# ai4co/rl4co

Hardware: NVIDIA H100
Metric: node-selections/sec TSP-100 AM rollout (higher is better)
Workload: dtype f32

## Files before the change

rl4co_b200/csrc/rollout_impl.cuh:

```cuda
#pragma once
#include "co_common.cuh"

namespace co {

#define CO_MODE_GREEDY 0
#define CO_MODE_SAMPLE 1
#define CO_MODE_EVALUATE 2

template <int SPL>
struct Cfg {
  static constexpr int NS = 32 * SPL;
  static constexpr int NW = SPL;
  static constexpr int MINB = SPL == 4 ? 1 : (SPL == 2 ? 2 : 3);
};

constexpr int TILE_LD = 20;

template <int SPL>
struct Smem {
  float ptab[(32 * SPL + 1) * E];
  float qfix[E];
  float wcap[E];
  float hfirst[E];
  float tile[8][32 * TILE_LD];
  alignas(16) float oh[8][D];
  alignas(16) float part[8][32 * SPL];
  alignas(16) float zbuf[2][32 * SPL];
  alignas(16) uint2 red[4];
  alignas(16) float lps[32];
  float dem[32 * SPL];
  float lim[32 * SPL];
  float2 loc[32 * SPL];
  unsigned char order[32 * SPL];
  unsigned char rank_of[32 * SPL];
  alignas(16) float wdyn[3 * E];
  alignas(16) float pwk[32 * SPL * 8 + 8];
};

__device__ __forceinline__ float ex2(float x) {
  float y;
  asm("ex2.approx.ftz.f32 %0, %1;" : "=f"(y) : "f"(x));
  return y;
}
__device__ __forceinline__ float lg2(float x) {
  float y;
  asm("lg2.approx.ftz.f32 %0, %1;" : "=f"(y) : "f"(x));
  return y;
}
__device__ __forceinline__ unsigned fkey(float f) {
  unsigned u = __float_as_uint(f);
  return u ^ ((u >> 31) ? 0xffffffffu : 0x80000000u);
}
__device__ __forceinline__ float funkey(unsigned k) {
  return __uint_as_float(k ^ ((k >> 31) ? 0x80000000u : 0xffffffffu));
}

__device__ __forceinline__ float warp_sum_fixed(float x) {
  constexpr float S = 16777216.f;
  const unsigned hi = __float2uint_rz(x * S);
  const float rem = fmaf(x, S, -(float)hi);
  const unsigned lo = __float2uint_rz(rem * S);
  const unsigned Hs = __reduce_add_sync(FULL, hi), Ls = __reduce_add_sync(FULL, lo);
  return fmaf((float)Ls, 1.0f / (S * S), (float)Hs * (1.0f / S));
}

static __device__ __noinline__ void first_node_gemv(const float* __restrict__ w_first, const float* hfirst, float* qfix, int tid) {
  const int e = tid >> 1, half = tid & 1;
  const float4* wr = reinterpret_cast<const float4*>(w_first + (size_t)e * E + 64 * half);
  const float4* hv = reinterpret_cast<const float4*>(hfirst + 64 * half);
  float s0 = 0.f, s1 = 0.f;
#pragma unroll
  for (int c = 0; c < 16; c += 2) {
    const float4 w0 = __ldg(wr + c), x0 = hv[c], w1 = __ldg(wr + c + 1), x1 = hv[c + 1];
    s0 = fmaf(w0.x, x0.x, s0); s0 = fmaf(w0.y, x0.y, s0); s0 = fmaf(w0.z, x0.z, s0); s0 = fmaf(w0.w, x0.w, s0);
    s1 = fmaf(w1.x, x1.x, s1); s1 = fmaf(w1.y, x1.y, s1); s1 = fmaf(w1.z, x1.z, s1); s1 = fmaf(w1.w, x1.w, s1);
  }
  float sacc = s0 + s1;
  sacc += __shfl_xor_sync(FULL, sacc, 1);
  if (half == 0) qfix[e] += sacc;
}

__device__ __forceinline__ float dist2_fma(float2 a, float2 b) {
  const float dx = a.x - b.x, dy = a.y - b.y;
  return sqrtf(fmaf(dy, dy, dx * dx));
}

template <int ENV>
__device__ __forceinline__ bool feasible(int n, bool visbit, float d, float used, float thr, int cur, bool anyfeas) {
  if (ENV == CO_ENV_TSP) return !visbit;
  if (ENV == CO_ENV_OP) return (n == 0) || (!visbit && !anyfeas && !(d > thr));
  if (ENV == CO_ENV_PCTSP) return (n == 0) ? !((used < 1.0f) && anyfeas) : (!visbit && d == 0.0f);
  if (n == 0) return !(cur == 0 && anyfeas);
  if (ENV == CO_ENV_SDVRP) return !visbit && !(d == 0.0f) && !(used >= thr);
  return !visbit && !((d + used) > thr);
}

template <int SPL, int ENV, int MODE, int CWB>
__global__ void __launch_bounds__(256, Cfg<SPL>::MINB) rollout_kernel(const co_rollout_args A) {
  using C = Cfg<SPL>;
  constexpr int NS = C::NS, NW = C::NW;
  constexpr int CW = CWB * E;
  constexpr int CUR_BLK = CWB - 1;
  constexpr bool first_table = (ENV == CO_ENV_TSP) && (CWB == 5);
  constexpr bool VRP = (ENV != CO_ENV_TSP);
  constexpr bool SD = (ENV == CO_ENV_SDVRP);
  constexpr bool OP = (ENV == CO_ENV_OP);
  constexpr bool PC = (ENV == CO_ENV_PCTSP);
  constexpr float LOG2E = 1.4426950408889634f, LN2 = 0.6931471805599453f;
  extern __shared__ __align__(16) unsigned char smem_raw[];
  Smem<SPL>& sm = *reinterpret_cast<Smem<SPL>*>(smem_raw);

  const int tid = threadIdx.x, lane = tid & 31, h = tid >> 5;
  const int N = A.N, B_inst = A.B_inst, S = A.num_starts, T_max = A.T_max;
  const int B_traj = B_inst * S;
  const bool forced_start = (S > 1) && (A.flags & CO_ROLLOUT_FORCED_START);
  const bool philox = (A.noise == nullptr);
  const bool sel_warp = h < NW;
  const bool lp_warp = h == NW;
  const int nL = sel_warp ? tid : NS - 1;
  const int nG = SPL * lane;
  const float clip = A.tanh_clipping, inv_temp = 1.0f / A.temperature;
  const float Zb = clip * inv_temp;
  float* tile = sm.tile[h];

  float2 Kr[SPL][8], Vr[SPL][8], Lr[SPL][8];

  for (int b = blockIdx.x; b < B_inst; b += gridDim.x) {
    __syncthreads();
    const float* crow = A.cache + (size_t)b * N * CW;
#pragma unroll
    for (int k = 0; k < SPL; ++k) {
      const int n = nG + k;
      if (n < N) {
        const float4* ks = reinterpret_cast<const float4*>(crow + (size_t)n * CW + 0 * E + h * D);
        const float4* vs = reinterpret_cast<const float4*>(crow + (size_t)n * CW + 1 * E + h * D);
        const float4* ls = reinterpret_cast<const float4*>(crow + (size_t)n * CW + 2 * E + h * D);
#pragma unroll
        for (int c = 0; c < 4; ++c) {
          const float4 kv = __ldg(ks + c), vv = __ldg(vs + c), lv = __ldg(ls + c);
          Kr[k][2 * c] = make_float2(kv.x, kv.y); Kr[k][2 * c + 1] = make_float2(kv.z, kv.w);
          Vr[k][2 * c] = make_float2(vv.x, vv.y); Vr[k][2 * c + 1] = make_float2(vv.z, vv.w);
          Lr[k][2 * c] = make_float2(lv.x, lv.y); Lr[k][2 * c + 1] = make_float2(lv.z, lv.w);
        }
      } else {
#pragma unroll
        for (int j = 0; j < 8; ++j) {
          Kr[k][j] = make_float2(0.f, 0.f); Vr[k][j] = make_float2(0.f, 0.f); Lr[k][j] = make_float2(0.f, 0.f);
        }
      }
    }
    for (int idx = tid; idx < N * (E / 4); idx += 256) {
      const int n = idx >> 5, c = idx & 31;
      const uint32_t dst = (uint32_t)__cvta_generic_to_shared(reinterpret_cast<float4*>(sm.ptab + n * E) + c);
      asm volatile("cp.async.cg.shared.global [%0], [%1], 16;" ::"r"(dst),
                   "l"(reinterpret_cast<const float4*>(crow + (size_t)n * CW + CUR_BLK * E) + c) : "memory");
    }
    asm volatile("cp.async.commit_group;" ::: "memory");
    if (tid < E) {
      sm.ptab[NS * E + tid] = 0.f;
      sm.wcap[tid] = VRP ? A.w_capacity[tid] : 0.f;
    }
    if (tid < NS) {
      sm.loc[tid] = (tid < N) ? reinterpret_cast<const float2*>(A.locs)[(size_t)b * N + tid] : make_float2(0.f, 0.f);
      sm.dem[tid] = (VRP && tid >= 1 && tid < N) ? A.demand[(size_t)b * (N - 1) + tid - 1] : 0.f;
      if (OP || PC) sm.lim[tid] = (tid < N) ? A.node_limit[(size_t)b * N + tid] : 0.f;
    }
    if (SD) {
      for (int i = tid; i < 3 * E; i += 256) sm.wdyn[i] = A.dyn_w[i];
    }
    const float cap = (VRP && A.vehicle_capacity) ? A.vehicle_capacity[b] : 1.0f;
    const float thr = SD ? cap : cap + 1e-5f;
    asm volatile("cp.async.wait_group 0;" ::: "memory");
    __syncthreads();
    if (SD) {
      for (int i = tid; i < (NS + 1) * 8; i += 256) {
        const int n = i >> 3, hh = i & 7;
        float acc = 0.f;
        if (n < N) {
#pragma unroll
          for (int c = 0; c < D; ++c) acc = fmaf(sm.ptab[n * E + hh * D + c], sm.wdyn[hh * D + c], acc);
        }
        sm.pwk[i] = acc;
      }
      __syncthreads();
    }
    if (ENV == CO_ENV_CVRP) {
      if (tid >= 1 && tid < N) {
        const float d = sm.dem[tid];
        int rank = 0;
        for (int m = 1; m < N; ++m) {
          const float dm = sm.dem[m];
          rank += (dm < d || (dm == d && m < tid)) ? 1 : 0;
        }
        sm.order[rank] = (unsigned char)tid;
        sm.rank_of[tid] = (unsigned char)rank;
      }
      __syncthreads();
    }
    float dmk0[SPL];
    float2 lck[SPL];
#pragma unroll
    for (int k = 0; k < SPL; ++k) {
      dmk0[k] = OP ? sm.lim[nG + k] : sm.dem[nG + k];
      lck[k] = OP ? sm.loc[nG + k] : make_float2(0.f, 0.f);
    }
    const float dL0 = OP ? sm.lim[nL] : sm.dem[nL];
    const float2 lcL = OP ? sm.loc[nL] : make_float2(0.f, 0.f);
    auto head_dot = [&](const float* vec, float (&out)[SPL]) {
      const float4* vp = reinterpret_cast<const float4*>(vec + h * D);
      float2 a2[SPL];
#pragma unroll
      for (int k = 0; k < SPL; ++k) a2[k] = make_float2(0.f, 0.f);
#pragma unroll
      for (int c = 0; c < 4; ++c) {
        const float4 x = vp[c];
#pragma unroll
        for (int k = 0; k < SPL; ++k) {
          a2[k] = ffma2(make_float2(x.x, x.y), Kr[k][2 * c], a2[k]);
          a2[k] = ffma2(make_float2(x.z, x.w), Kr[k][2 * c + 1], a2[k]);
        }
      }
#pragma unroll
      for (int k = 0; k < SPL; ++k) out[k] = a2[k].x + a2[k].y;
    };
    auto add_first = [&](int a_first) {
      if (first_table) {
        if (tid < E) sm.qfix[tid] += __ldg(crow + (size_t)a_first * CW + 3 * E + tid);
      } else {
        if (tid < E) sm.hfirst[tid] = __ldg(A.node_emb + ((size_t)b * N + a_first) * E + tid);
        __syncthreads();
        first_node_gemv(A.w_first, sm.hfirst, sm.qfix, tid);
      }
    };
    float WK[SPL], FK[SPL];
#pragma unroll
    for (int k = 0; k < SPL; ++k) { WK[k] = 0.f; FK[k] = 0.f; }
    if (VRP) head_dot(sm.wcap, WK);
    float WKW = 0.f, wv_d = 0.f;
    if (SD) {
#pragma unroll
      for (int c = 0; c < D; ++c) WKW = fmaf(sm.wcap[h * D + c], sm.wdyn[h * D + c], WKW);
      wv_d = sm.wdyn[E + h * D + (lane & 15)];
    }
    if (!(A.flags & CO_ROLLOUT_NO_PREFETCH) && b + (int)gridDim.x < B_inst) {
      const char* nxt = reinterpret_cast<const char*>(A.cache + (size_t)(b + gridDim.x) * N * CW);
      for (int i = tid; i < N * 16; i += 256) {
        const int n = i >> 4, blk = (i >> 2) & 3, line = i & 3;
        const size_t off = ((size_t)n * CW + (blk < 3 ? blk : CUR_BLK) * E) * 4 + ((size_t)line << 7);
        asm volatile("prefetch.global.L2 [%0];" ::"l"(nxt + off));
      }
    }

    for (int s = 0; s < S; ++s) {
      const int traj = s * B_inst + b;
      int64_t* act_row = A.actions_out + (size_t)traj * T_max;
      float* lp_row = A.logp_out + (size_t)traj * T_max;
      uint32_t mybits = (!sel_warp || nL >= N) ? 0x100u : 0u;
#pragma unroll
      for (int k = 0; k < SPL; ++k) mybits |= (nG + k >= N) ? (1u << k) : 0u;
      int cur = (ENV == CO_ENV_TSP) ? NS : 0;
      int prev = 0, first = 0, t = 0, dstep = 0, nvis = 0;
      uint32_t rmask[SPL];
#pragma unroll
      for (int k = 0; k < SPL; ++k) {
        const int lo = 32 * k, nc = N - 1;
        rmask[k] = (nc >= lo + 32) ? 0u : (nc <= lo ? 0xffffffffu : (0xffffffffu << (nc - lo)));
      }
      float used = 0.f, dist = 0.f;
      bool anyfeas = false, done = false, depot_seen = false;
      float dmk[SPL], dL = dL0;
#pragma unroll
      for (int k = 0; k < SPL; ++k) dmk[k] = dmk0[k];
      int nrem = 0;
      int pend_a = -1;
      float pend_d = 0.f, FKW = 0.f;
      float ll = 0.f;
      float pen = 0.f;
      if (SD && s > 0 && tid < NS) sm.dem[tid] = (tid >= 1 && tid < N) ? A.demand[(size_t)b * (N - 1) + tid - 1] : 0.f;
      __syncthreads();
      if (tid < E) {
        float g = A.graph_ctx ? A.graph_ctx[(size_t)b * E + tid] : 0.f;
        if (ENV == CO_ENV_TSP && !forced_start) g += A.q_placeholder[tid];
        sm.qfix[tid] = g;
      }

      auto env_step = [&](int a) {
        if (!SD) {
          const unsigned dd = (unsigned)(a - nG);
          mybits |= (dd < (unsigned)SPL) ? (1u << dd) : 0u;
          mybits |= (a == nL) ? 0x100u : 0u;
        }
        if (!OP && h == 0) {
          const float2 pa = sm.loc[a], pp = sm.loc[prev];
          const float dx = pa.x - pp.x, dy = pa.y - pp.y;
          if (VRP || t != 0) dist += sqrtf(dx * dx + dy * dy);
        }
        if (ENV == CO_ENV_TSP) {
          if (t == 0) first = a;
        } else if (OP) {
          used = used + dist2_fma(sm.loc[a], sm.loc[prev]);
          if (h == 0) dist += sm.dem[a];
          depot_seen = depot_seen || (a == 0);
        } else if (PC) {
          used = used + sm.dem[a];
          if (h == 0) pen += sm.lim[a];
          nvis += (a != 0) ? 1 : 0;
          depot_seen = depot_seen || (a == 0);
        } else if (SD) {
          const float d_a = sm.dem[a];
          const float delivered = fminf(d_a, cap - used);
          used = (used + delivered) * (a != 0 ? 1.0f : 0.0f);
          const float d_new = d_a + (-delivered);
#pragma unroll
          for (int k = 0; k < SPL; ++k) dmk[k] = (a == nG + k) ? d_new : dmk[k];
          dL = (a == nL) ? d_new : dL;
          nrem += ((d_new > 0.f) ? 1 : 0) - ((d_a > 0.f) ? 1 : 0);
          pend_a = a; pend_d = d_new;
          anyfeas = (nrem > 0) && !(used >= cap);
        } else {
          used = (used + sm.dem[a == 0 ? 1 : a]) * (a != 0 ? 1.0f : 0.0f);
          nvis += (a != 0 || !depot_seen) ? 1 : 0;
          depot_seen = depot_seen || (a == 0);
          if (a != 0) {
            const int r = sm.rank_of[a];
#pragma unroll
            for (int k = 0; k < SPL; ++k) rmask[k] |= ((r >> 5) == k) ? (1u << (r & 31)) : 0u;
          }
          int pmin = NS;
#pragma unroll
          for (int k = SPL - 1; k >= 0; --k) {
            const uint32_t z = ~rmask[k];
            if (z) pmin = 32 * k + __ffs(z) - 1;
          }
          anyfeas = (pmin < N - 1) && !((sm.dem[sm.order[pmin < N - 1 ? pmin : 0]] + used) > thr);
        }
        prev = a; cur = a; ++t;
        done = (ENV == CO_ENV_TSP) ? (t >= N) : ((OP || PC) ? (a == 0 && t > 1) : (SD ? (nrem == 0) : (nvis >= N)));
      };
      auto logp_of = [&](int buf, int a_sel, int t_out) {
        const float* zb = sm.zbuf[buf];
        float sacc = 0.f;
#pragma unroll
        for (int k = 0; k < SPL; ++k) sacc += ex2((zb[nG + k] - Zb) * LOG2E);
        sm.lps[lane] = sacc;
        __syncwarp();
        const float4* lq = reinterpret_cast<const float4*>(sm.lps);
        const float4 q0 = lq[0], q1 = lq[1], q2 = lq[2], q3 = lq[3], q4 = lq[4], q5 = lq[5], q6 = lq[6], q7 = lq[7];
        const float t0 = ((q0.x + q0.y) + (q0.z + q0.w)) + ((q1.x + q1.y) + (q1.z + q1.w));
        const float t1 = ((q2.x + q2.y) + (q2.z + q2.w)) + ((q3.x + q3.y) + (q3.z + q3.w));
        const float t2 = ((q4.x + q4.y) + (q4.z + q4.w)) + ((q5.x + q5.y) + (q5.z + q5.w));
        const float t3 = ((q6.x + q6.y) + (q6.z + q6.w)) + ((q7.x + q7.y) + (q7.z + q7.w));
        sacc = (t0 + t1) + (t2 + t3);
        __syncwarp();
        const float lp = (zb[a_sel] - Zb) - lg2(sacc) * LN2;
        if (lane == 0) {
          lp_row[t_out] = lp;
          ll += lp;
        }
      };

      if (SD) {
        for (int n = 1; n < N; ++n) nrem += (sm.dem[n] > 0.f) ? 1 : 0;
        anyfeas = (nrem > 0) && !(used >= cap);
        done = (nrem == 0);
      }
      if (forced_start) {
        const int a0 = (s % A.num_loc) + (VRP ? 1 : 0);
        if (tid == 0) { act_row[0] = a0; lp_row[0] = 0.f; }
        env_step(a0);
        if (ENV == CO_ENV_TSP) {
          __syncthreads();
          add_first(a0);
        }
      } else if (ENV == CO_ENV_CVRP) {
        anyfeas = !((sm.dem[sm.order[0]] + used) > thr);
      }
      __syncthreads();
      head_dot(sm.qfix, FK);
      if (SD) {
#pragma unroll
        for (int c = 0; c < D; ++c) FKW = fmaf(sm.qfix[h * D + c], sm.wdyn[h * D + c], FKW);
      }

      while (!done && t < T_max) {
        int forced = 0;
        float gum = 0.f;
        if (MODE == CO_MODE_EVALUATE) forced = (int)A.forced_actions[(size_t)traj * T_max + t];
        if (MODE == CO_MODE_SAMPLE && tid < N) {
          const float q = philox ? philox_exp1(A.seed, A.offset, traj, dstep, tid)
                                 : A.noise[((size_t)dstep * B_traj + traj) * N + tid];
          gum = -logf(q);
        }

        {
          const float4* pr = reinterpret_cast<const float4*>(sm.ptab + cur * E + h * D);
          const float rem = PC ? fmaxf(cap - used, 0.0f) : cap - used;
          float2 sc2[SPL];
#pragma unroll
          for (int k = 0; k < SPL; ++k) sc2[k] = make_float2(0.f, 0.f);
#pragma unroll
          for (int c = 0; c < 4; ++c) {
            const float4 p = pr[c];
#pragma unroll
            for (int k = 0; k < SPL; ++k) {
              sc2[k] = ffma2(make_float2(p.x, p.y), Kr[k][2 * c], sc2[k]);
              sc2[k] = ffma2(make_float2(p.z, p.w), Kr[k][2 * c + 1], sc2[k]);
            }
          }
          float sc[SPL], m = -INFINITY;
          bool fz[SPL];
          const float qwk = SD ? fmaf(rem, WKW, sm.pwk[cur * 8 + h] + FKW) : 0.f;
          const float2 pcur = OP ? sm.loc[cur] : make_float2(0.f, 0.f);
#pragma unroll
          for (int k = 0; k < SPL; ++k) {
            fz[k] = OP ? feasible<ENV>(nG + k, (mybits >> k) & 1u, used + dist2_fma(lck[k], pcur), used, dmk[k], cur, depot_seen)
                    : PC ? feasible<ENV>(nG + k, (mybits >> k) & 1u, depot_seen ? 1.0f : 0.0f, used, thr, cur, nvis < N - 1)
                         : feasible<ENV>(nG + k, (mybits >> k) & 1u, dmk[k], used, thr, cur, anyfeas);
            float dot = (sc2[k].x + sc2[k].y) + FK[k];
            if (VRP) dot = fmaf(rem, WK[k], dot);
            if (SD) dot = fmaf(dmk[k], qwk, dot);
            sc[k] = fz[k] ? dot * (0.25f * LOG2E) : -INFINITY;
            m = fmaxf(m, sc[k]);
          }
          m = funkey(__reduce_max_sync(FULL, fkey(m)));
          float2 acc[8];
          float esum = 0.f, sed = 0.f;
#pragma unroll
          for (int j = 0; j < 8; ++j) acc[j] = make_float2(0.f, 0.f);
#pragma unroll
          for (int k = 0; k < SPL; ++k) {
            const float e = fz[k] ? ex2(sc[k] - m) : 0.f;
            esum += e;
            if (SD) sed = fmaf(e, dmk[k], sed);
            const float2 e2 = make_float2(e, e);
#pragma unroll
            for (int j = 0; j < 8; ++j) acc[j] = ffma2(e2, Vr[k][j], acc[j]);
          }
          float4* trow = reinterpret_cast<float4*>(tile + lane * TILE_LD);
#pragma unroll
          for (int c = 0; c < 4; ++c) trow[c] = make_float4(acc[2 * c].x, acc[2 * c].y, acc[2 * c + 1].x, acc[2 * c + 1].y);
          if (SD) sed = warp_sum(sed);
          __syncwarp();
          const int d = lane & 15, half = lane >> 4;
          float s0 = 0.f, s1 = 0.f, s2 = 0.f, s3 = 0.f;
#pragma unroll
          for (int r = 0; r < 16; r += 4) {
            s0 += tile[(16 * half + ((r + 0 + 4 * half) & 15)) * TILE_LD + d];
            s1 += tile[(16 * half + ((r + 1 + 4 * half) & 15)) * TILE_LD + d];
            s2 += tile[(16 * half + ((r + 2 + 4 * half) & 15)) * TILE_LD + d];
            s3 += tile[(16 * half + ((r + 3 + 4 * half) & 15)) * TILE_LD + d];
          }
          float r = (s0 + s1) + (s2 + s3);
          r += __shfl_xor_sync(FULL, r, 16);
          if (SD) r = fmaf(sed, wv_d, r);
          if (lane < 16) sm.oh[h][lane] = r;
          __syncwarp();
          const float4* op = reinterpret_cast<const float4*>(sm.oh[h]);
          float2 pl2[SPL];
          float olh = 0.f;
#pragma unroll
          for (int k = 0; k < SPL; ++k) pl2[k] = make_float2(0.f, 0.f);
#pragma unroll
          for (int c = 0; c < 4; ++c) {
            const float4 x = op[c];
#pragma unroll
            for (int k = 0; k < SPL; ++k) {
              pl2[k] = ffma2(make_float2(x.x, x.y), Lr[k][2 * c], pl2[k]);
              pl2[k] = ffma2(make_float2(x.z, x.w), Lr[k][2 * c + 1], pl2[k]);
            }
            if (SD) {
              const float4 w = reinterpret_cast<const float4*>(sm.wdyn + 2 * E + h * D)[c];
              olh = fmaf(x.x, w.x, olh); olh = fmaf(x.y, w.y, olh); olh = fmaf(x.z, w.z, olh); olh = fmaf(x.w, w.w, olh);
            }
          }
          esum = warp_sum_fixed(esum);
          const float rinv = __fdividef(1.0f, esum);
          float pl[SPL];
#pragma unroll
          for (int k = 0; k < SPL; ++k) {
            float v = pl2[k].x + pl2[k].y;
            if (SD) v = fmaf(dmk[k], olh, v);
            pl[k] = v * rinv;
          }
          float* pdst = sm.part[h] + nG;
          if (SPL == 4) *reinterpret_cast<float4*>(pdst) = make_float4(pl[0], pl[SPL > 1 ? 1 : 0], pl[SPL > 2 ? 2 : 0], pl[SPL > 3 ? 3 : 0]);
          else if (SPL == 2) *reinterpret_cast<float2*>(pdst) = make_float2(pl[0], pl[SPL > 1 ? 1 : 0]);
          else *pdst = pl[0];
        }
        __syncthreads();

        if (SD && tid == 0 && pend_a >= 0) sm.dem[pend_a] = pend_d;
        if (sel_warp) {
          const bool fzL = OP ? feasible<ENV>(nL, (mybits >> 8) & 1u, used + dist2_fma(lcL, sm.loc[cur]), used, dL, cur, depot_seen)
                           : PC ? feasible<ENV>(nL, (mybits >> 8) & 1u, depot_seen ? 1.0f : 0.0f, used, thr, cur, nvis < N - 1)
                                : feasible<ENV>(nL, (mybits >> 8) & 1u, dL, used, thr, cur, anyfeas);
          const float p = ((sm.part[0][nL] + sm.part[1][nL]) + (sm.part[2][nL] + sm.part[3][nL])) +
                          ((sm.part[4][nL] + sm.part[5][nL]) + (sm.part[6][nL] + sm.part[7][nL]));
          const float lg = tanhf(p * 0.08838834764831845f) * clip;
          const float z = fzL ? lg * inv_temp : -INFINITY;
          sm.zbuf[dstep & 1][nL] = z;
          if (MODE != CO_MODE_EVALUATE) {
            const float keyf = (MODE == CO_MODE_SAMPLE) ? (fzL ? z + gum : -INFINITY) : z;
            const unsigned key = fkey(keyf);
            const unsigned wkey = __reduce_max_sync(FULL, key);
            const unsigned vote = __ballot_sync(FULL, key == wkey);
            if (lane == 0) sm.red[h] = make_uint2(wkey, (unsigned)(32 * h + __ffs(vote) - 1));
          }
        } else if (lp_warp && dstep > 0) {
          logp_of((dstep - 1) & 1, prev, t - 1);
        }
        __syncthreads();
        int a;
        if (MODE == CO_MODE_EVALUATE) {
          a = (forced < 0 || forced >= N) ? 0 : forced;
        } else if (NW == 1) {
          a = (int)sm.red[0].y;
        } else if (NW == 2) {
          const uint4 r0 = reinterpret_cast<const uint4*>(sm.red)[0];
          a = (int)((r0.z > r0.x) ? r0.w : r0.y);
        } else {
          const uint4 r0 = reinterpret_cast<const uint4*>(sm.red)[0], r1 = reinterpret_cast<const uint4*>(sm.red)[1];
          const bool b01 = r0.z > r0.x, b23 = r1.z > r1.x;
          const unsigned ka = b01 ? r0.z : r0.x, ia = b01 ? r0.w : r0.y;
          const unsigned kb = b23 ? r1.z : r1.x, ib = b23 ? r1.w : r1.y;
          a = (int)((kb > ka) ? ib : ia);
        }
        if (tid == 0) act_row[t] = a;

        const bool was_first = (ENV == CO_ENV_TSP) && (t == 0);
        env_step(a);
        ++dstep;
        if (was_first) {
          if (tid < E) sm.qfix[tid] = A.graph_ctx ? A.graph_ctx[(size_t)b * E + tid] : 0.f;
          __syncthreads();
          add_first(a);
          __syncthreads();
          head_dot(sm.qfix, FK);
        }
      }

      __syncthreads();
      if (lp_warp) {
        if (dstep > 0) logp_of((dstep - 1) & 1, prev, t - 1);
        if (lane == 0) A.loglik_out[traj] = ll;
      }
      if (tid == 0) {
        const float2 pa = sm.loc[(ENV == CO_ENV_TSP) ? first : 0], pp = sm.loc[prev];
        const float dx = pa.x - pp.x, dy = pa.y - pp.y;
        float rw = OP ? dist : -(dist + sqrtf(dx * dx + dy * dy));
        if (PC) {
          float total = 0.f;
          for (int n = 1; n < N; ++n) total += sm.lim[n];
          rw = pen - (-rw + total);
        }
        A.reward_out[traj] = rw;
        if (A.steps_out) A.steps_out[traj] = t;
        if (A.used_capacity_out) A.used_capacity_out[traj] = used;
        if (A.max_steps_out) atomicMax(A.max_steps_out, t);
      }
      for (int c = t + tid; c < T_max; c += 256) { act_row[c] = 0; lp_row[c] = 0.f; }
    }
  }
}

template <int SPL, int ENV, int MODE, int CWB>
static int launch(const co_rollout_args& A, cudaStream_t st) {
  auto kern = rollout_kernel<SPL, ENV, MODE, CWB>;
  const size_t smem = sizeof(Smem<SPL>);
  static PerDeviceOnce once;
  static int ctas_per_sm = 1;
  bool& configured = once.flag();
  if (!configured) {
    cudaError_t e = cudaFuncSetAttribute(kern, cudaFuncAttributeMaxDynamicSharedMemorySize, (int)smem);
    if (e != cudaSuccess) return fail(CO_ERR_CUDA, "co_rollout: smem attribute: %s", cudaGetErrorString(e));
    e = cudaOccupancyMaxActiveBlocksPerMultiprocessor(&ctas_per_sm, kern, 256, smem);
    if (e != cudaSuccess || ctas_per_sm < 1) return fail(CO_ERR_CUDA, "co_rollout: occupancy query failed%s");
    configured = true;
  }
  int grid = device_info().sm_count * ctas_per_sm;
  if (grid > A.B_inst) grid = A.B_inst;
  kern<<<grid, 256, smem, st>>>(A);
  return check_launch("co_rollout");
}

template <int ENV>
static int dispatch(const co_rollout_args& A, cudaStream_t st) {
  const int spl = A.N <= 32 ? 1 : (A.N <= 64 ? 2 : 4);
  const int mode = A.select_mode == CO_SELECT_GREEDY ? CO_MODE_GREEDY
                   : (A.select_mode == CO_SELECT_EVALUATE ? CO_MODE_EVALUATE : CO_MODE_SAMPLE);
  const int cwb = A.cache_width / E;
#define CO_CASE(S_, M_)                                                                      \
  if (spl == S_ && mode == M_) {                                                             \
    if (cwb == 4) return launch<S_, ENV, M_, 4>(A, st);                                      \
    if (ENV == CO_ENV_TSP && cwb == 5) return launch<S_, ENV, M_, (ENV == CO_ENV_TSP ? 5 : 4)>(A, st); \
  }
  CO_CASE(1, CO_MODE_GREEDY) CO_CASE(2, CO_MODE_GREEDY) CO_CASE(4, CO_MODE_GREEDY)
  CO_CASE(1, CO_MODE_SAMPLE) CO_CASE(2, CO_MODE_SAMPLE) CO_CASE(4, CO_MODE_SAMPLE)
  CO_CASE(1, CO_MODE_EVALUATE) CO_CASE(2, CO_MODE_EVALUATE) CO_CASE(4, CO_MODE_EVALUATE)
#undef CO_CASE
  return fail(CO_ERR_BAD_ARG, "co_rollout: no kernel variant%s");
}

}
```

rl4co_b200/csrc/rollout_tsp.cu:

```cuda
#include "rollout_impl.cuh"
namespace co {
int rollout_tsp(const co_rollout_args& A, cudaStream_t st) { return dispatch<CO_ENV_TSP>(A, st); }
}
```

rl4co_b200/native.py:

```python

from __future__ import annotations

import ctypes
import os
import subprocess
import sys
from ctypes import POINTER, Structure, c_char_p, c_float, c_int, c_int32, c_uint64, c_void_p

import torch

_HERE = os.path.dirname(os.path.abspath(__file__))
CSRC = os.path.join(_HERE, "csrc")
INCLUDE = os.path.join(os.path.dirname(_HERE), "include")
LIB_PATH = os.path.join(_HERE, "libcorollout.so")
SOURCES = ["abi.cu", "env_kernels.cu", "decode_step.cu", "rollout.cu", "rollout_tsp.cu", "rollout_cvrp.cu", "rollout_ms_tsp.cu", "rollout_ms_cvrp.cu", "rollout_sdvrp.cu", "rollout_op.cu", "rollout_pctsp.cu", "gemm_tf32x3.cu",
           "encoder_mha.cu", "encoder_mha_wgmma.cu",
           "ffn_fused.cu", "data_kernels.cu", "attn_train.cu", "norm_kernels.cu", "op_kernels.cu", "local_search.cu", "eas_kernels.cu"]
HEADERS = ["co_common.cuh", "rollout_impl.cuh", "rollout_ms_impl.cuh", "wgmma.cuh"]

CO_OK = 0
ENV_TSP, ENV_CVRP = 0, 1
ENV_SDVRP = 2
ENV_OP, ENV_PCTSP = 3, 4
ENV_KIND = {"tsp": ENV_TSP, "cvrp": ENV_CVRP, "sdvrp": ENV_SDVRP, "op": ENV_OP, "pctsp": ENV_PCTSP}
ROLLOUT_ENVS = ("tsp", "cvrp", "sdvrp", "op", "pctsp")
SELECT_GREEDY, SELECT_SAMPLE_NOISE, SELECT_EVALUATE, SELECT_SAMPLE_PHILOX = 0, 1, 2, 3
ROLLOUT_FORCED_START = 1
EMBED_DIM, NUM_HEADS = 128, 8

EXPORTS = [
    "co_version", "co_last_error_string", "co_device_sm_count", "co_tsp_step", "co_cvrp_action_mask",
    "co_cvrp_step", "co_tour_length", "co_check_tours", "co_pointer_logits", "co_select_action",
    "co_cache_width", "co_rollout_max_nodes", "co_rollout", "co_reward_stats", "co_split_tf32", "co_gemm_tf32x3", "co_encoder_mha",
    "co_ffn_fused", "co_ffn_tile_weights", "co_ffn_tiled_weight_floats", "co_generate_uniform", "co_generate_demand", "co_dihedral8",
    "co_sdvrp_step", "co_sdvrp_action_mask", "co_attn_fwd", "co_attn_bwd", "co_instance_norm", "co_op_step", "co_op_action_mask", "co_op_reward", "co_pctsp_step", "co_pctsp_action_mask",
    "co_tsp_two_opt", "co_generate_locs", "co_symmetric_augment", "co_cvrp_local_search",
    "co_eas_key_grad",
]


class NativeLibraryError(RuntimeError):
    pass


class DecoderWeights(Structure):
    _fields_ = [("project_context_t", c_void_p), ("w_placeholder", c_void_p), ("project_out_t", c_void_p),
                ("dynamic_w", c_void_p), ("dynamic_feature", c_void_p)]


class RolloutArgs(Structure):
    _fields_ = [
        ("env_kind", c_int32), ("select_mode", c_int32), ("B_inst", c_int32), ("num_starts", c_int32),
        ("N", c_int32), ("T_max", c_int32), ("num_loc", c_int32), ("flags", c_int32),
        ("tanh_clipping", c_float), ("temperature", c_float),
        ("cache", c_void_p), ("graph_ctx", c_void_p), ("q_placeholder", c_void_p), ("w_capacity", c_void_p),
        ("locs", c_void_p), ("demand", c_void_p), ("vehicle_capacity", c_void_p),
        ("forced_actions", c_void_p), ("noise", c_void_p), ("seed", c_uint64), ("offset", c_uint64),
        ("actions_out", c_void_p), ("logp_out", c_void_p), ("reward_out", c_void_p), ("loglik_out", c_void_p),
        ("steps_out", c_void_p), ("max_steps_out", c_void_p), ("used_capacity_out", c_void_p),
        ("node_emb", c_void_p), ("w_first", c_void_p), ("cache_width", c_int32), ("reserved0", c_int32),
        ("dyn_w", c_void_p), ("node_limit", c_void_p),
    ]


class EasGradArgs(Structure):
    _fields_ = [("env_kind", c_int32), ("B_inst", c_int32), ("num_rows", c_int32), ("N", c_int32), ("T", c_int32),
                ("cache_width", c_int32), ("tanh_clipping", c_float), ("temperature", c_float)] + [
        (n, c_void_p) for n in ("cache", "graph_ctx", "w_capacity", "demand", "vehicle_capacity", "actions", "coef",
                                "dLf", "loglik", "bad_rows")]


class AttnArgs(Structure):
    _fields_ = ([(n, c_void_p) for n in ("q", "k", "v", "mask", "o", "lse", "dO", "dq", "dk", "dv")]
                + [(n, c_int32) for n in ("B", "M", "N", "reserved0")]
                + [(n, ctypes.c_int64) for n in ("q_bs", "k_bs", "v_bs", "o_bs", "dq_bs", "dk_bs", "dv_bs")]
                + [(n, c_int32) for n in ("q_rs", "k_rs", "v_rs", "o_rs", "dq_rs", "dk_rs", "dv_rs")]
                + [("scale", c_float)])


class LocsArgs(Structure):
    _fields_ = [("B", ctypes.c_int64), ("N", c_int32), ("kind", c_int32), ("seed", c_uint64), ("offset", c_uint64),
                ("lo", c_float), ("hi", c_float), ("mean", c_float), ("std", c_float), ("n_cluster", c_int32),
                ("n_cluster_mix", c_int32), ("num_modes", c_int32), ("cdist", c_float)]


LOCS_KIND = {"uniform": 0, "constant": 1, "normal": 2, "cluster": 3, "mixed": 4, "gaussian_mixture": 5,
             "mix_distribution": 6, "mix_multi_distributions": 7}
LOCS_MAX_NODES = 10000


NVCC_FLAGS = ["-gencode", "arch=compute_90a,code=sm_90a", "-O3", "-lineinfo", "-std=c++17",
              "-Xcompiler", "-fPIC", "-I", INCLUDE]


def _nvcc() -> str:
    nvcc = os.environ.get("NVCC", "/usr/local/cuda/bin/nvcc")
    return nvcc if os.path.exists(nvcc) else "nvcc"


def build(force: bool = False, verbose: bool = False, extra_flags: list[str] | None = None) -> str:
    deps = [os.path.join(CSRC, s) for s in SOURCES + HEADERS] + [os.path.join(INCLUDE, "corollout.h")]
    if not force and os.path.exists(LIB_PATH) and all(os.path.getmtime(LIB_PATH) >= os.path.getmtime(s) for s in deps):
        return LIB_PATH
    objdir = os.path.join(_HERE, "build")
    os.makedirs(objdir, exist_ok=True)
    procs = []
    for s in SOURCES:
        obj = os.path.join(objdir, s.replace(".cu", ".o"))
        cmd = [_nvcc()] + NVCC_FLAGS + (extra_flags or []) + ["-c", os.path.join(CSRC, s), "-o", obj]
        if verbose:
            print(" ".join(cmd), file=sys.stderr)
        procs.append((s, obj, subprocess.Popen(cmd, stdout=subprocess.PIPE, stderr=subprocess.STDOUT, text=True)))
    objs, log = [], []
    for s, obj, p in procs:
        out, _ = p.communicate()
        log.append(out)
        if p.returncode != 0:
            raise NativeLibraryError(f"nvcc failed on {s} ({p.returncode}):\n{out}")
        objs.append(obj)
    link = [_nvcc(), "-gencode", "arch=compute_90a,code=sm_90a", "-shared", "-o", LIB_PATH] + objs
    res = subprocess.run(link, capture_output=True, text=True)
    if res.returncode != 0:
        raise NativeLibraryError(f"link failed ({res.returncode}):\n{res.stdout}\n{res.stderr}")
    build.last_log = "\n".join(log)
    return LIB_PATH


_lib = None


def lib() -> ctypes.CDLL:
    global _lib
    if _lib is not None:
        return _lib
    if not os.path.exists(LIB_PATH):
        raise NativeLibraryError(
            f"{LIB_PATH} not found: run `python -c 'import __graft_entry__ as g; g.build()'` "
            "(there is no CPU/PyTorch fallback for the rollout path)")
    L = ctypes.CDLL(LIB_PATH)
    for name in EXPORTS:
        if not hasattr(L, name):
            raise NativeLibraryError(f"{LIB_PATH} does not export {name}")
    L.co_last_error_string.restype = c_char_p
    L.co_rollout.argtypes = [POINTER(RolloutArgs), c_void_p]
    L.co_pointer_logits.argtypes = [c_int, POINTER(DecoderWeights)] + [c_void_p] * 12 + [c_int, c_int, c_int, c_int, c_void_p]
    L.co_select_action.argtypes = [c_void_p] * 6 + [c_int, c_float, c_float, c_int, c_uint64, c_uint64, c_int, c_int, c_void_p]
    L.co_tsp_step.argtypes = [c_void_p] * 7 + [c_int, c_int, c_void_p]
    L.co_cvrp_action_mask.argtypes = [c_void_p] * 6 + [c_int, c_int, c_void_p]
    L.co_cvrp_step.argtypes = [c_void_p] * 10 + [c_int, c_int, c_void_p]
    L.co_tour_length.argtypes = [c_void_p] * 3 + [c_int] * 5 + [c_void_p]
    L.co_sdvrp_action_mask.argtypes = [c_void_p] * 5 + [c_int, c_int, c_void_p]
    L.co_sdvrp_step.argtypes = [c_void_p] * 9 + [c_int, c_int, c_void_p]
    L.co_check_tours.argtypes = [c_void_p] * 4 + [c_int] * 4 + [c_void_p]
    L.co_tsp_two_opt.argtypes = [c_void_p] * 5 + [c_int] * 3 + [c_void_p]
    L.co_cvrp_local_search.argtypes = [c_void_p] * 9 + [c_int] * 4 + [c_void_p]
    L.co_reward_stats.argtypes = [c_void_p, c_void_p, c_int, c_void_p]
    L.co_op_action_mask.argtypes = [c_void_p] * 6 + [c_int, c_int, c_void_p]
    L.co_op_step.argtypes = [c_void_p] * 12 + [c_int, c_int, c_void_p]
    L.co_pctsp_action_mask.argtypes = [c_void_p] * 3 + [c_int, c_int, c_void_p]
    L.co_pctsp_step.argtypes = [c_void_p] * 11 + [c_int, c_int, c_void_p]
    L.co_op_reward.argtypes = [c_void_p] * 3 + [c_int, c_int, c_int, c_void_p]
    L.co_instance_norm.argtypes = [c_void_p, c_void_p, c_void_p, c_void_p, ctypes.c_long, c_int, c_float, c_void_p]
    L.co_eas_key_grad.argtypes = [POINTER(EasGradArgs), c_void_p]
    L.co_attn_fwd.argtypes = [POINTER(AttnArgs), c_void_p]
    L.co_attn_bwd.argtypes = [POINTER(AttnArgs), c_void_p]
    L.co_cache_width.argtypes = [c_int]
    L.co_split_tf32.argtypes = [c_void_p, c_void_p, c_void_p, ctypes.c_long, c_void_p]
    L.co_gemm_tf32x3.argtypes = [c_void_p] * 8 + [c_int] * 7 + [c_void_p]
    L.co_encoder_mha.argtypes = [c_void_p, c_void_p, c_int, c_int, c_void_p]
    L.co_ffn_fused.argtypes = [c_void_p] * 7 + [c_int, c_int, c_int, c_void_p]
    L.co_ffn_tile_weights.argtypes = [c_void_p] * 5 + [c_void_p]
    L.co_ffn_tiled_weight_floats.restype = ctypes.c_long
    L.co_generate_uniform.argtypes = [c_void_p, ctypes.c_long, c_uint64, c_uint64, c_float, c_float, c_void_p]
    L.co_generate_demand.argtypes = [c_void_p, ctypes.c_long, c_uint64, c_uint64, c_int, c_int, c_float, c_void_p]
    L.co_dihedral8.argtypes = [c_void_p, c_void_p, ctypes.c_long, c_int, c_void_p]
    L.co_symmetric_augment.argtypes = [c_void_p, c_void_p, c_void_p, ctypes.c_long, c_int, c_int, c_void_p]
    L.co_generate_locs.argtypes = [c_void_p, POINTER(LocsArgs), c_void_p]
    _lib = L
    return L


LAUNCH_COUNT = 0


def _check(rc: int, what: str) -> None:
    global LAUNCH_COUNT
    LAUNCH_COUNT += 1
    if rc != CO_OK:
        msg = lib().co_last_error_string().decode("utf-8", "replace")
        raise NativeLibraryError(f"{what} failed with code {rc}: {msg}")


def _ptr(t: torch.Tensor | None, dtype: torch.dtype | None = None, name: str = "tensor", strided: bool = False):
    if t is None:
        return None
    if not isinstance(t, torch.Tensor):
        raise TypeError(f"{name}: expected a torch.Tensor, got {type(t)}")
    if not t.is_cuda:
        raise NativeLibraryError(f"{name}: libcorollout needs CUDA tensors (got device {t.device}); "
                                 "there is no CPU fallback")
    if dtype is not None and t.dtype != dtype:
        raise TypeError(f"{name}: expected dtype {dtype}, got {t.dtype}")
    if not strided and not t.is_contiguous():
        raise ValueError(f"{name}: tensor must be contiguous")
    return t.data_ptr()


def _stream():
    return torch.cuda.current_stream().cuda_stream


def _on_device_of_first_tensor(fn):
    import functools

    @functools.wraps(fn)
    def wrapper(*args, **kwargs):
        for a in list(args) + list(kwargs.values()):
            if isinstance(a, torch.Tensor) and a.is_cuda:
                if a.device.index != torch.cuda.current_device():
                    with torch.cuda.device(a.device):
                        return fn(*args, **kwargs)
                break
        return fn(*args, **kwargs)

    return wrapper


F32, I64, U8, I32 = torch.float32, torch.int64, torch.uint8, torch.int32


def _bool_ptr(t, name):
    if t is None:
        return None
    if t.dtype not in (torch.bool, torch.uint8):
        raise TypeError(f"{name}: expected bool/uint8, got {t.dtype}")
    return _ptr(t, None, name)




def version() -> int:
    return lib().co_version()


def cache_width(env_name: str) -> int:
    return lib().co_cache_width(ENV_KIND[env_name])


def rollout_max_nodes() -> int:
    return lib().co_rollout_max_nodes()


@_on_device_of_first_tensor
def tsp_step(action, mask_in, mask_out, first_node, current_node, i, done):
    B, N = mask_in.shape
    _check(lib().co_tsp_step(_ptr(action, I64, "action"), _bool_ptr(mask_in, "mask_in"), _bool_ptr(mask_out, "mask_out"),
                             _ptr(first_node, I64, "first_node"), _ptr(current_node, I64, "current_node"),
                             _ptr(i, I64, "i"), _bool_ptr(done, "done"), B, N, _stream()), "co_tsp_step")


@_on_device_of_first_tensor
def cvrp_action_mask(demand, used, cap, visited, current_node, mask_out):
    B, N = visited.shape
    _check(lib().co_cvrp_action_mask(_ptr(demand, F32, "demand"), _ptr(used, F32, "used"), _ptr(cap, F32, "cap"),
                                     _ptr(visited, U8, "visited"), _ptr(current_node, I64, "current_node"),
                                     _bool_ptr(mask_out, "mask_out"), B, N, _stream()), "co_cvrp_action_mask")


@_on_device_of_first_tensor
def cvrp_step(action, demand, cap, used_in, used_out, visited_in, visited_out, current_node, done, mask_out):
    B, N = visited_in.shape
    _check(lib().co_cvrp_step(_ptr(action, I64, "action"), _ptr(demand, F32, "demand"), _ptr(cap, F32, "cap"),
                              _ptr(used_in, F32, "used_in"), _ptr(used_out, F32, "used_out"),
                              _ptr(visited_in, U8, "visited_in"), _ptr(visited_out, U8, "visited_out"),
                              _ptr(current_node, I64, "current_node"), _bool_ptr(done, "done"),
                              _bool_ptr(mask_out, "mask_out"), B, N, _stream()), "co_cvrp_step")


@_on_device_of_first_tensor
def sdvrp_action_mask(demand_with_depot, used, cap, current_node, mask_out):
    B, N = demand_with_depot.shape
    _check(lib().co_sdvrp_action_mask(_ptr(demand_with_depot, F32, "demand_with_depot"), _ptr(used, F32, "used_capacity"),
                                      _ptr(cap, F32, "vehicle_capacity"), _ptr(current_node, I64, "current_node"),
                                      _bool_ptr(mask_out, "mask_out"), B, N, _stream()), "co_sdvrp_action_mask")
    return mask_out


@_on_device_of_first_tensor
def sdvrp_step(action, demand_in, demand_out, cap, used_in, used_out, current_node, done, mask_out):
    B, N = demand_in.shape
    _check(lib().co_sdvrp_step(_ptr(action, I64, "action"), _ptr(demand_in, F32, "demand_in"),
                               _ptr(demand_out, F32, "demand_out"), _ptr(cap, F32, "vehicle_capacity"),
                               _ptr(used_in, F32, "used_in"), _ptr(used_out, F32, "used_out"),
                               _ptr(current_node, I64, "current_node"), _bool_ptr(done, "done"),
                               _bool_ptr(mask_out, "mask_out"), B, N, _stream()), "co_sdvrp_step")


@_on_device_of_first_tensor
def op_action_mask(locs, max_length, visited, tour_length, current_node, mask_out):
    B, N = mask_out.shape
    _check(lib().co_op_action_mask(_ptr(locs, F32, "locs"), _ptr(max_length, F32, "max_length"), _bool_ptr(visited, "visited"),
                                   _ptr(tour_length, F32, "tour_length"), _ptr(current_node, I64, "current_node"),
                                   _bool_ptr(mask_out, "mask_out"), B, N, _stream()), "co_op_action_mask")
    return mask_out


@_on_device_of_first_tensor
def op_step(action, locs, prize, max_length, visited_in, visited_out, tour_length, current_total_prize, current_node, i,
            done, mask_out):
    B, N = mask_out.shape
    _check(lib().co_op_step(_ptr(action, I64, "action"), _ptr(locs, F32, "locs"), _ptr(prize, F32, "prize"),
                            _ptr(max_length, F32, "max_length"), _bool_ptr(visited_in, "visited_in"),
                            _bool_ptr(visited_out, "visited_out"), _ptr(tour_length, F32, "tour_length"),
                            _ptr(current_total_prize, F32, "current_total_prize"), _ptr(current_node, I64, "current_node"),
                            _ptr(i, I64, "i"), _bool_ptr(done, "done"), _bool_ptr(mask_out, "mask_out"), B, N, _stream()),
           "co_op_step")


@_on_device_of_first_tensor
def pctsp_action_mask(visited, cur_total_prize, mask_out):
    B, N = mask_out.shape
    _check(lib().co_pctsp_action_mask(_bool_ptr(visited, "visited"), _ptr(cur_total_prize, F32, "cur_total_prize"),
                                      _bool_ptr(mask_out, "mask_out"), B, N, _stream()), "co_pctsp_action_mask")
    return mask_out


@_on_device_of_first_tensor
def pctsp_step(action, real_prize, penalty, visited_in, visited_out, cur_total_prize, cur_total_penalty, current_node, i, done,
               mask_out):
    B, N = mask_out.shape
    _check(lib().co_pctsp_step(_ptr(action, I64, "action"), _ptr(real_prize, F32, "real_prize"), _ptr(penalty, F32, "penalty"),
                               _bool_ptr(visited_in, "visited_in"), _bool_ptr(visited_out, "visited_out"),
                               _ptr(cur_total_prize, F32, "cur_total_prize"), _ptr(cur_total_penalty, F32, "cur_total_penalty"),
                               _ptr(current_node, I64, "current_node"), _ptr(i, I64, "i"), _bool_ptr(done, "done"),
                               _bool_ptr(mask_out, "mask_out"), B, N, _stream()), "co_pctsp_step")


@_on_device_of_first_tensor
def op_reward(prize, actions):
    B, T = actions.shape
    if prize.shape[0] != B:
        prize = prize.repeat(B // prize.shape[0], 1)
    out = torch.empty(B, dtype=F32, device=actions.device)
    _check(lib().co_op_reward(_ptr(prize.contiguous(), F32, "prize"), _ptr(actions, I64, "actions"), _ptr(out, F32, "reward"),
                              B, prize.shape[1], T, _stream()), "co_op_reward")
    return out


@_on_device_of_first_tensor
def tour_length(locs, actions, with_depot: bool):
    B, T = actions.shape
    B_locs, N = locs.shape[0], locs.shape[1]
    reward = torch.empty(B, dtype=F32, device=actions.device)
    _check(lib().co_tour_length(_ptr(locs, F32, "locs"), _ptr(actions, I64, "actions"), _ptr(reward, F32, "reward"),
                                B, B_locs, N, T, int(with_depot), _stream()), "co_tour_length")
    return reward


@_on_device_of_first_tensor
def check_tours(actions, N, demand=None, cap=None, B_inst=None) -> int:
    B, T = actions.shape
    bad = torch.zeros(1, dtype=I32, device=actions.device)
    _check(lib().co_check_tours(_ptr(actions, I64, "actions"), _ptr(demand, F32, "demand"), _ptr(cap, F32, "cap"),
                                _ptr(bad, I32, "bad"), B, B if B_inst is None else B_inst, N, T, _stream()),
           "co_check_tours")
    return int(bad.item())


@_on_device_of_first_tensor
def tsp_two_opt(tours, max_iterations: int = 1000, locs=None, distances=None, iterations=None):
    if (locs is None) == (distances is None):
        raise ValueError("tsp_two_opt: pass exactly one of locs / distances")
    if tours.dim() != 2:
        raise ValueError(f"tours: expected [B, N], got {tuple(tours.shape)}")
    B, N = tours.shape
    if locs is not None and tuple(locs.shape) != (B, N, 2):
        raise ValueError(f"locs: expected [{B}, {N}, 2], got {tuple(locs.shape)}")
    if distances is not None and tuple(distances.shape) != (B, N, N):
        raise ValueError(f"distances: expected [{B}, {N}, {N}], got {tuple(distances.shape)}")
    if iterations is not None and tuple(iterations.shape) != (B,):
        raise ValueError(f"iterations: expected [{B}], got {tuple(iterations.shape)}")
    out = torch.empty(B, N, dtype=I64, device=tours.device)
    _check(lib().co_tsp_two_opt(_ptr(locs, F32, "locs"), _ptr(distances, F32, "distances"), _ptr(tours, I64, "tours"),
                                _ptr(out, I64, "tours_out"), _ptr(iterations, I32, "iterations"), B, N,
                                min(int(max_iterations), 2**31 - 1), _stream()), "co_tsp_two_opt")
    return out


@_on_device_of_first_tensor
def cvrp_local_search(tours, demand, capacity, max_iterations: int, locs=None, distances=None, iterations=None,
                      feasible=None):
    if (locs is None) == (distances is None):
        raise ValueError("cvrp_local_search: pass exactly one of locs / distances")
    if tours.dim() != 2:
        raise ValueError(f"tours: expected [B, T], got {tuple(tours.shape)}")
    B, T = tours.shape
    if demand.dim() != 2 or demand.shape[0] != B:
        raise ValueError(f"demand: expected [{B}, N], got {tuple(demand.shape)}")
    N = demand.shape[1]
    if tuple(capacity.shape) != (B,):
        raise ValueError(f"capacity: expected [{B}], got {tuple(capacity.shape)}")
    if locs is not None and tuple(locs.shape) != (B, N + 1, 2):
        raise ValueError(f"locs: expected [{B}, {N + 1}, 2], got {tuple(locs.shape)}")
    if distances is not None and tuple(distances.shape) != (B, N + 1, N + 1):
        raise ValueError(f"distances: expected [{B}, {N + 1}, {N + 1}], got {tuple(distances.shape)}")
    for name, t in (("iterations", iterations), ("feasible", feasible)):
        if t is not None and tuple(t.shape) != (B,):
            raise ValueError(f"{name}: expected [{B}], got {tuple(t.shape)}")
    out = torch.empty(B, 2 * N, dtype=I64, device=tours.device)
    used = torch.empty(B, dtype=I32, device=tours.device)
    _check(lib().co_cvrp_local_search(_ptr(locs, F32, "locs"), _ptr(distances, F32, "distances"),
                                      _ptr(demand, F32, "demand"), _ptr(capacity, F32, "capacity"),
                                      _ptr(tours, I64, "tours"), _ptr(out, I64, "tours_out"), _ptr(used, I32, "used"),
                                      _ptr(iterations, I32, "iterations"), _ptr(feasible, I32, "feasible"), B, N, T,
                                      min(int(max_iterations), 2**31 - 1), _stream()), "co_cvrp_local_search")
    return out, used


@_on_device_of_first_tensor
def eas_key_grad(env_name, cache, actions, coef, graph_ctx=None, w_capacity=None, demand=None, vehicle_capacity=None,
                 tanh_clipping=10.0, temperature=1.0, bad_rows=None):
    if env_name not in ("tsp", "cvrp"):
        raise NotImplementedError(f"co_eas_key_grad covers tsp and cvrp, not {env_name!r}")
    if cache.dim() != 3:
        raise ValueError(f"cache: expected [B_inst, N, W], got {tuple(cache.shape)}")
    B_inst, N, W = cache.shape
    if actions.dim() != 2 or B_inst == 0 or actions.shape[0] % max(B_inst, 1) or actions.shape[0] == 0:
        raise ValueError(f"actions: expected [R * {B_inst}, T], got {tuple(actions.shape)}")
# ... 310 lines not shown
```

Baseline: 103.6 million.

## Offload per-step bookkeeping and log-prob finish to dedicated spare warps

Moves tour-length accounting, action stores and penalty accumulation out of the critical env_step path into a separate bookkeeping warp that runs one step behind. Log-prob computation is split into partials (lp warp) and a finish stage (another warp) running two steps behind, with double-buffered shared state. The aim is to shorten the serial per-step path that warp 0 and the selection warps wait on, using otherwise idle warps. It also adds optional clock64 phase-timing instrumentation behind a compile flag, plus a configurable library path for the build. The tail handling after the loop gains an extra __syncthreads and drain logic, which adds complexity.

```diff
diff --git a/rl4co_b200/csrc/rollout_impl.cuh b/rl4co_b200/csrc/rollout_impl.cuh
--- a/rl4co_b200/csrc/rollout_impl.cuh
+++ b/rl4co_b200/csrc/rollout_impl.cuh
@@ -27,7 +27,10 @@
   alignas(16) float part[8][32 * SPL];
   alignas(16) float zbuf[2][32 * SPL];
   alignas(16) uint2 red[4];
-  alignas(16) float lps[32];
+  alignas(16) float lps[2][32];
+  float lsel[2];
+  float ll;
+  float pen;
   float dem[32 * SPL];
   float lim[32 * SPL];
   float2 loc[32 * SPL];
@@ -36,6 +39,16 @@
   alignas(16) float wdyn[3 * E];
   alignas(16) float pwk[32 * SPL * 8 + 8];
 };
+
+#ifdef CO_PHASE_CLOCKS
+static __constant__ unsigned long long* co_phase_clk;
+#define CO_PHASE_STAMP(row, slot)                                                                    \
+  do {                                                                                               \
+    if (lane == 0) co_phase_clk[(((size_t)b * T_max + (row)) * 8 + h) * 6 + (slot)] = clock64();   \
+  } while (0)
+#else
+#define CO_PHASE_STAMP(row, slot) do { } while (0)
+#endif
 
 __device__ __forceinline__ float ex2(float x) {
   float y;
@@ -117,6 +130,8 @@
   const bool philox = (A.noise == nullptr);
   const bool sel_warp = h < NW;
   const bool lp_warp = h == NW;
+  const bool bk_warp = h == NW + 1;
+  const bool ll_warp = h == NW + 2;
   const int nL = sel_warp ? tid : NS - 1;
   const int nG = SPL * lane;
   const float clip = A.tanh_clipping, inv_temp = 1.0f / A.temperature;
@@ -126,6 +141,7 @@
   float2 Kr[SPL][8], Vr[SPL][8], Lr[SPL][8];
 
   for (int b = blockIdx.x; b < B_inst; b += gridDim.x) {
+    CO_PHASE_STAMP(0, 5);
     __syncthreads();
     const float* crow = A.cache + (size_t)b * N * CW;
 #pragma unroll
@@ -253,20 +269,21 @@
 
     for (int s = 0; s < S; ++s) {
       const int traj = s * B_inst + b;
-      int64_t* act_row = A.actions_out + (size_t)traj * T_max;
-      float* lp_row = A.logp_out + (size_t)traj * T_max;
+      const size_t row = (size_t)traj * T_max;
       uint32_t mybits = (!sel_warp || nL >= N) ? 0x100u : 0u;
 #pragma unroll
       for (int k = 0; k < SPL; ++k) mybits |= (nG + k >= N) ? (1u << k) : 0u;
       int cur = (ENV == CO_ENV_TSP) ? NS : 0;
-      int prev = 0, first = 0, t = 0, dstep = 0, nvis = 0;
+      int first = 0, t = 0, dstep = 0, nvis = 0;
+      int prev = 0;
+      float dist = 0.f;
       uint32_t rmask[SPL];
 #pragma unroll
       for (int k = 0; k < SPL; ++k) {
         const int lo = 32 * k, nc = N - 1;
         rmask[k] = (nc >= lo + 32) ? 0u : (nc <= lo ? 0xffffffffu : (0xffffffffu << (nc - lo)));
       }
-      float used = 0.f, dist = 0.f;
+      float used = 0.f;
       bool anyfeas = false, done = false, depot_seen = false;
       float dmk[SPL], dL = dL0;
 #pragma unroll
@@ -274,10 +291,10 @@
       int nrem = 0;
       int pend_a = -1;
       float pend_d = 0.f, FKW = 0.f;
-      float ll = 0.f;
-      float pen = 0.f;
       if (SD && s > 0 && tid < NS) sm.dem[tid] = (tid >= 1 && tid < N) ? A.demand[(size_t)b * (N - 1) + tid - 1] : 0.f;
       __syncthreads();
+      if (bk_warp && lane == 0) sm.pen = 0.f;
+      if (ll_warp && lane == 0) sm.ll = 0.f;
       if (tid < E) {
         float g = A.graph_ctx ? A.graph_ctx[(size_t)b * E + tid] : 0.f;
         if (ENV == CO_ENV_TSP && !forced_start) g += A.q_placeholder[tid];
@@ -290,20 +307,13 @@
           mybits |= (dd < (unsigned)SPL) ? (1u << dd) : 0u;
           mybits |= (a == nL) ? 0x100u : 0u;
         }
-        if (!OP && h == 0) {
-          const float2 pa = sm.loc[a], pp = sm.loc[prev];
-          const float dx = pa.x - pp.x, dy = pa.y - pp.y;
-          if (VRP || t != 0) dist += sqrtf(dx * dx + dy * dy);
-        }
         if (ENV == CO_ENV_TSP) {
           if (t == 0) first = a;
         } else if (OP) {
-          used = used + dist2_fma(sm.loc[a], sm.loc[prev]);
-          if (h == 0) dist += sm.dem[a];
+          used = used + dist2_fma(sm.loc[a], sm.loc[cur]);
           depot_seen = depot_seen || (a == 0);
         } else if (PC) {
           used = used + sm.dem[a];
-          if (h == 0) pen += sm.lim[a];
           nvis += (a != 0) ? 1 : 0;
           depot_seen = depot_seen || (a == 0);
         } else if (SD) {
@@ -334,29 +344,43 @@
           }
           anyfeas = (pmin < N - 1) && !((sm.dem[sm.order[pmin < N - 1 ? pmin : 0]] + used) > thr);
         }
-        prev = a; cur = a; ++t;
+        cur = a; ++t;
         done = (ENV == CO_ENV_TSP) ? (t >= N) : ((OP || PC) ? (a == 0 && t > 1) : (SD ? (nrem == 0) : (nvis >= N)));
       };
-      auto logp_of = [&](int buf, int a_sel, int t_out) {
+      auto logp_partials = [&](int buf) {
         const float* zb = sm.zbuf[buf];
         float sacc = 0.f;
 #pragma unroll
         for (int k = 0; k < SPL; ++k) sacc += ex2((zb[nG + k] - Zb) * LOG2E);
-        sm.lps[lane] = sacc;
-        __syncwarp();
-        const float4* lq = reinterpret_cast<const float4*>(sm.lps);
+        sm.lps[buf][lane] = sacc;
+        if (lane == 0) sm.lsel[buf] = zb[cur] - Zb;
+      };
+      auto logp_finish = [&](int buf, int t_out) {
+        const float ll_prev = sm.ll;
+        const float4* lq = reinterpret_cast<const float4*>(sm.lps[buf]);
         const float4 q0 = lq[0], q1 = lq[1], q2 = lq[2], q3 = lq[3], q4 = lq[4], q5 = lq[5], q6 = lq[6], q7 = lq[7];
         const float t0 = ((q0.x + q0.y) + (q0.z + q0.w)) + ((q1.x + q1.y) + (q1.z + q1.w));
         const float t1 = ((q2.x + q2.y) + (q2.z + q2.w)) + ((q3.x + q3.y) + (q3.z + q3.w));
         const float t2 = ((q4.x + q4.y) + (q4.z + q4.w)) + ((q5.x + q5.y) + (q5.z + q5.w));
         const float t3 = ((q6.x + q6.y) + (q6.z + q6.w)) + ((q7.x + q7.y) + (q7.z + q7.w));
-        sacc = (t0 + t1) + (t2 + t3);
-        __syncwarp();
-        const float lp = (zb[a_sel] - Zb) - lg2(sacc) * LN2;
+        const float sacc = (t0 + t1) + (t2 + t3);
+        const float lp = sm.lsel[buf] - lg2(sacc) * LN2;
         if (lane == 0) {
-          lp_row[t_out] = lp;
-          ll += lp;
-        }
+          sm.ll = ll_prev + lp;
+          A.logp_out[row + t_out] = lp;
+        }
+      };
+      auto account = [&](int a, int ta) {
+        if (!OP) {
+          const float2 pa = sm.loc[a], pp = sm.loc[prev];
+          const float dx = pa.x - pp.x, dy = pa.y - pp.y;
+          const float leg = sqrtf(dx * dx + dy * dy);
+          dist += (VRP || ta != 0) ? leg : 0.f;
+        }
+        if (OP) dist += sm.dem[a];
+        if (PC && lane == 0) sm.pen += sm.lim[a];
+        if (lane == 0) A.actions_out[row + ta] = a;
+        prev = a;
       };
 
       if (SD) {
@@ -366,8 +390,9 @@
       }
       if (forced_start) {
         const int a0 = (s % A.num_loc) + (VRP ? 1 : 0);
-        if (tid == 0) { act_row[0] = a0; lp_row[0] = 0.f; }
+        if (tid == 0) A.logp_out[row] = 0.f;
         env_step(a0);
+        if (bk_warp) account(a0, 0);
         if (ENV == CO_ENV_TSP) {
           __syncthreads();
           add_first(a0);
@@ -383,6 +408,7 @@
       }
 
       while (!done && t < T_max) {
+        CO_PHASE_STAMP(dstep, 0);
         int forced = 0;
         float gum = 0.f;
         if (MODE == CO_MODE_EVALUATE) forced = (int)A.forced_actions[(size_t)traj * T_max + t];
@@ -487,7 +513,9 @@
           else if (SPL == 2) *reinterpret_cast<float2*>(pdst) = make_float2(pl[0], pl[SPL > 1 ? 1 : 0]);
           else *pdst = pl[0];
         }
+        CO_PHASE_STAMP(dstep, 1);
         __syncthreads();
+        CO_PHASE_STAMP(dstep, 2);
 
         if (SD && tid == 0 && pend_a >= 0) sm.dem[pend_a] = pend_d;
         if (sel_warp) {
@@ -506,10 +534,16 @@
             const unsigned vote = __ballot_sync(FULL, key == wkey);
             if (lane == 0) sm.red[h] = make_uint2(wkey, (unsigned)(32 * h + __ffs(vote) - 1));
           }
+        } else if (bk_warp) {
+          if (dstep > 0) account(cur, t - 1);
+        } else if (ll_warp) {
+          if (dstep > 1) logp_finish(dstep & 1, t - 2);
         } else if (lp_warp && dstep > 0) {
-          logp_of((dstep - 1) & 1, prev, t - 1);
-        }
+          logp_partials((dstep - 1) & 1);
+        }
+        CO_PHASE_STAMP(dstep, 3);
         __syncthreads();
+        CO_PHASE_STAMP(dstep, 4);
         int a;
         if (MODE == CO_MODE_EVALUATE) {
           a = (forced < 0 || forced >= N) ? 0 : forced;
@@ -525,7 +559,6 @@
           const unsigned kb = b23 ? r1.z : r1.x, ib = b23 ? r1.w : r1.y;
           a = (int)((kb > ka) ? ib : ia);
         }
-        if (tid == 0) act_row[t] = a;
 
         const bool was_first = (ENV == CO_ENV_TSP) && (t == 0);
         env_step(a);
@@ -540,25 +573,28 @@
       }
 
       __syncthreads();
-      if (lp_warp) {
-        if (dstep > 0) logp_of((dstep - 1) & 1, prev, t - 1);
-        if (lane == 0) A.loglik_out[traj] = ll;
-      }
-      if (tid == 0) {
+      if (lp_warp && dstep > 0) logp_partials((dstep - 1) & 1);
+      __syncthreads();
+      if (ll_warp) {
+        for (int k = dstep > 1 ? dstep - 2 : 0; k < dstep; ++k) logp_finish(k & 1, t - dstep + k);
+        if (lane == 0) A.loglik_out[traj] = sm.ll;
+      }
+      if (bk_warp && dstep > 0) account(cur, t - 1);
+      if (bk_warp && lane == 0) {
         const float2 pa = sm.loc[(ENV == CO_ENV_TSP) ? first : 0], pp = sm.loc[prev];
         const float dx = pa.x - pp.x, dy = pa.y - pp.y;
         float rw = OP ? dist : -(dist + sqrtf(dx * dx + dy * dy));
         if (PC) {
           float total = 0.f;
           for (int n = 1; n < N; ++n) total += sm.lim[n];
-          rw = pen - (-rw + total);
+          rw = sm.pen - (-rw + total);
         }
         A.reward_out[traj] = rw;
         if (A.steps_out) A.steps_out[traj] = t;
         if (A.used_capacity_out) A.used_capacity_out[traj] = used;
         if (A.max_steps_out) atomicMax(A.max_steps_out, t);
       }
-      for (int c = t + tid; c < T_max; c += 256) { act_row[c] = 0; lp_row[c] = 0.f; }
+      for (int c = t + tid; c < T_max; c += 256) { A.actions_out[row + c] = 0; A.logp_out[row + c] = 0.f; }
     }
   }
 }
diff --git a/rl4co_b200/csrc/rollout_tsp.cu b/rl4co_b200/csrc/rollout_tsp.cu
--- a/rl4co_b200/csrc/rollout_tsp.cu
+++ b/rl4co_b200/csrc/rollout_tsp.cu
@@ -2,3 +2,9 @@
 namespace co {
 int rollout_tsp(const co_rollout_args& A, cudaStream_t st) { return dispatch<CO_ENV_TSP>(A, st); }
 }
+
+#ifdef CO_PHASE_CLOCKS
+extern "C" int co_phase_clocks_set(void* buf) {
+  return cudaMemcpyToSymbol(co::co_phase_clk, &buf, sizeof(buf)) == cudaSuccess ? 0 : 1;
+}
+#endif
diff --git a/rl4co_b200/native.py b/rl4co_b200/native.py
--- a/rl4co_b200/native.py
+++ b/rl4co_b200/native.py
@@ -98,11 +98,12 @@
     return nvcc if os.path.exists(nvcc) else "nvcc"
 
 
-def build(force: bool = False, verbose: bool = False, extra_flags: list[str] | None = None) -> str:
+def build(force: bool = False, verbose: bool = False, extra_flags: list[str] | None = None,
+          lib_path: str = LIB_PATH) -> str:
     deps = [os.path.join(CSRC, s) for s in SOURCES + HEADERS] + [os.path.join(INCLUDE, "corollout.h")]
-    if not force and os.path.exists(LIB_PATH) and all(os.path.getmtime(LIB_PATH) >= os.path.getmtime(s) for s in deps):
-        return LIB_PATH
-    objdir = os.path.join(_HERE, "build")
+    if not force and os.path.exists(lib_path) and all(os.path.getmtime(lib_path) >= os.path.getmtime(s) for s in deps):
+        return lib_path
+    objdir = os.path.join(os.path.dirname(os.path.abspath(lib_path)), "build")
     os.makedirs(objdir, exist_ok=True)
     procs = []
     for s in SOURCES:
@@ -118,12 +119,12 @@
         if p.returncode != 0:
             raise NativeLibraryError(f"nvcc failed on {s} ({p.returncode}):\n{out}")
         objs.append(obj)
-    link = [_nvcc(), "-gencode", "arch=compute_90a,code=sm_90a", "-shared", "-o", LIB_PATH] + objs
+    link = [_nvcc(), "-gencode", "arch=compute_90a,code=sm_90a", "-shared", "-o", lib_path] + objs
     res = subprocess.run(link, capture_output=True, text=True)
     if res.returncode != 0:
         raise NativeLibraryError(f"link failed ({res.returncode}):\n{res.stdout}\n{res.stderr}")
     build.last_log = "\n".join(log)
-    return LIB_PATH
+    return lib_path
 
 
 _lib = None
```

Measured after the change: 108.2 million (median of 6 runs). 1.04x the previous value.
